# RtrMmmt/MPI-BiCGStab

Hardware: NVIDIA H100
Metric: BiCGStab iterations/sec (higher is better)
Workload: dtype f64

## Files before the change

mpi-bicgstab_b200/csrc/engine.hpp:

```cpp
#pragma once
#include "bicgstab_b200.h"
#include "dev.cuh"
#include "plan.hpp"
#include "spmv.cuh"
#include "vec.cuh"
#include "mega.cuh"

#include <cstdio>
#include <cstdlib>
#include <functional>
#include <initializer_list>
#include <map>
#include <string>
#include <vector>

namespace bicg {

[[noreturn]] void fatal(const char *fmt, ...);
#define BICG_CUDA(call)                                                                              \
    do {                                                                                             \
        cudaError_t e_ = (call);                                                                     \
        if (e_ != cudaSuccess)                                                                       \
            ::bicg::fatal("bicgstab_b200: CUDA error %s at %s:%d: %s", cudaGetErrorName(e_), __FILE__, \
                          __LINE__, cudaGetErrorString(e_));                                          \
// ... 74 lines not shown
    std::vector<Deferred> deferred;
    std::multimap<size_t, void *> pool;
    std::map<void *, size_t> live;
    size_t pool_bytes = 0;
    struct ArenaRec { char *ptr; size_t bytes; unsigned long long id; cudaIpcMemHandle_t handle; };
    std::multimap<size_t, ArenaRec> arena_pool;
    std::map<std::pair<int, unsigned long long>, void *> peer_maps;
    unsigned long long next_arena_id = 1;
    void release_arenas();
    void host_allgather(const void *send, void *recv, size_t bytes);
    void h2d(void *dst, const void *src, size_t bytes);
    struct Stager { cudaStream_t st = nullptr; cudaEvent_t ev[2] = {nullptr, nullptr}; cudaEvent_t done = nullptr; char *buf[2] = {nullptr, nullptr}; };
    std::vector<Stager> stagers;
    int stage_threads = 4;
};
Context &ctx();
void load_config_from_env(Config &c);
int  set_option(Config &c, const char *key, const char *value);


struct SpmvPlan {
    int kind = 0, lanes = 1, threads = 256, stages = 3, cap = 0, grid = 0, ctas_per_sm = 1;
    size_t smem = 0;
    int ntiles = 0;
    int *d_tile_row = nullptr;
    unsigned *d_tile_nz = nullptr;
    double ms = 0.0;
};

struct MegaPlan {
    bool ok = false;
    int threads = 512, lanes = 1, stages = 2, cap = 0, grid = 0;
    size_t smem = 0;
    size_t res_smem = 0;
    int ntiles = 0;
    int *d_tile_row = nullptr;
    unsigned *d_tile_nz = nullptr;
    int *d_cta_tile = nullptr;
    int4 *d_cta_dep = nullptr;
    unsigned short *d_col16 = nullptr;
    bool stream_codes = true;
    int *d_tile_flag = nullptr;
    bool chunked = false;
    std::vector<int> cta_row;
};

}

struct bicg_matrix {
    int rank = 0, world = 1;
    int n_loc = 0, n_glob = 0;
    size_t nnz = 0;
    unsigned max_row = 0;
    double mean_row = 0.0;
    double *d_val = nullptr;
    unsigned *d_col = nullptr;
    unsigned *d_ptr = nullptr;
    bicg::SpmvPlan plan;
    bicg::MegaPlan mega;
    bicg::MegaSync *d_msync = nullptr;
    bicg::MegaSync *peer_msync[bicg::MAX_RANKS] = {};
    unsigned long long *d_ll = nullptr;
    long long ll_stride = 0;
    unsigned long long *peer_ll[bicg::MAX_RANKS] = {};
    long long peer_ll_stride[bicg::MAX_RANKS] = {};
    unsigned long long *d_trace = nullptr;
    int ghost_off = 0;
    int n_ghost = 0;
    long long vstride = 0;
    std::vector<int> recv_runs;
    char *arena = nullptr;
    size_t arena_bytes = 0;
    unsigned long long arena_id = 0;
// ... 73 lines not shown
```

mpi-bicgstab_b200/csrc/matrix.cu:

```cuda
#include "engine.hpp"

#include <algorithm>
#include <climits>
#include <cmath>
#include <cstdarg>
#include <cstring>
#include <ctime>
#include <thread>

namespace bicg {

void fatal(const char *fmt, ...)
{
    va_list ap;
    va_start(ap, fmt);
    vfprintf(stderr, fmt, ap);
    va_end(ap);
    fputc('\n', stderr);
    exit(1);
}

namespace {

enum class Parse { Int, Double, Spmv };
// ... 431 lines not shown
    if (mean_row <= 20.0) return 1;
    if (mean_row <= 40.0) return 4;
    if (mean_row <= 128.0) return 8;
    return 32;
}

static void build_mega_plan(bicg_matrix *m, const unsigned *h_ptr, const std::vector<unsigned char> &row_extra)
{
    Context &c = ctx();
    MegaPlan &mp = m->mega;
    mp.ok = false;
    if (m->n_loc < 1) return;
    const int G = std::min(c.sm_count, MEGA_MAX_CTAS);
    const long long SMEM_MAX = 222 * 1024;
    const int lanes = c.cfg.mega_lanes > 0 ? c.cfg.mega_lanes : mega_lanes_for(m->mean_row);
    if (lanes != 1 && c.cfg.mega != 2 && c.cfg.mega_lanes == 0) return;
    for (int threads : {512, 256}) {
        if (c.cfg.mega_threads && c.cfg.mega_threads != threads) continue;
        if (!mega_has_variant(threads, lanes)) continue;
        const int rpt = threads / lanes;
        std::vector<int> tile_row, cta_tile, tile_flag;
        std::vector<unsigned> tile_nz;
        const int cap_limit = (int)(((SMEM_MAX / 2 - (long long)(rpt + 8) * 4) / 12) / 32 * 32) - 64;
        const unsigned max_tile_nnz = plan_cta_tiles(h_ptr, m->n_loc, G, rpt, row_extra.empty() ? nullptr : row_extra.data(),
                                                     c.cfg.boundary_weight, tile_row, cta_tile, cap_limit, &tile_nz, &tile_flag, c.cfg.row_weight);
        const int cap = round_up((long long)max_tile_nnz + 16, 32);
        const long long stage = (long long)cap * 12 + (long long)(rpt + 8) * 4;
        int stages = (int)std::min<long long>(4, SMEM_MAX / stage);
        if (stages < 2) continue;
        bool chunked = false;
        for (int f : tile_flag) chunked = chunked || f != 0;
        mp.chunked = chunked;
        mp.threads = threads; mp.lanes = lanes; mp.stages = stages; mp.cap = cap; mp.grid = G;
        mp.smem = mega_smem_bytes(cap, stages, threads, lanes);
        mp.res_smem = 0;
        if (lanes == 1 && !chunked) {
            size_t need = 0;
            for (int g = 0; g < G; ++g) {
                const int r0 = tile_row[(size_t)cta_tile[(size_t)g]], r1 = tile_row[(size_t)cta_tile[(size_t)g + 1]];
                need = std::max(need, mega_resident_bytes(h_ptr[r1] - h_ptr[r0], r1 - r0));
            }
            if (need <= (size_t)SMEM_MAX) mp.res_smem = std::max<size_t>(need, 16);
        }
        mp.ntiles = (int)tile_row.size() - 1;
        mp.cta_row.assign((size_t)G + 1, m->n_loc);
        for (int g = 0; g <= G; ++g) mp.cta_row[(size_t)g] = tile_row[(size_t)cta_tile[(size_t)g]];
        mp.d_tile_row = (decltype(mp.d_tile_row))c.dev_alloc(tile_row.size() * sizeof(int));
        mp.d_tile_nz = (decltype(mp.d_tile_nz))c.dev_alloc(tile_nz.size() * sizeof(unsigned));
        mp.d_cta_tile = (decltype(mp.d_cta_tile))c.dev_alloc(cta_tile.size() * sizeof(int));
        mp.d_cta_dep = (decltype(mp.d_cta_dep))c.dev_alloc((size_t)G * sizeof(int4));
        mp.d_tile_flag = nullptr;
        if (chunked) {
            mp.d_tile_flag = (int *)c.dev_alloc(tile_flag.size() * sizeof(int));
            BICG_CUDA(cudaMemcpy(mp.d_tile_flag, tile_flag.data(), tile_flag.size() * sizeof(int), cudaMemcpyHostToDevice));
        }
        BICG_CUDA(cudaMemcpy(mp.d_tile_row, tile_row.data(), tile_row.size() * sizeof(int), cudaMemcpyHostToDevice));
        BICG_CUDA(cudaMemcpy(mp.d_tile_nz, tile_nz.data(), tile_nz.size() * sizeof(unsigned), cudaMemcpyHostToDevice));
        BICG_CUDA(cudaMemcpy(mp.d_cta_tile, cta_tile.data(), cta_tile.size() * sizeof(int), cudaMemcpyHostToDevice));
        launch_mega_dep(m->d_col, m->d_ptr, mp.d_tile_row, mp.d_cta_tile, G, m->ghost_off, mp.d_cta_dep, c.stream);
        BICG_CUDA(cudaGetLastError());
        const size_t pad = 16;
        mp.d_col16 = (unsigned short *)c.dev_alloc((m->nnz + pad) * sizeof(unsigned short));
        BICG_CUDA(cudaMemsetAsync(mp.d_col16 + m->nnz, 0, pad * sizeof(unsigned short), c.stream));
        launch_mega_code(m->d_col, m->d_ptr, mp.d_tile_row, mp.d_cta_tile, G, m->ghost_off, mp.d_cta_dep, mp.d_col16, c.stream);
        BICG_CUDA(cudaGetLastError());
        mp.ok = true;
        if (c.cfg.verbose)
            fprintf(stderr, "[bicg mega r%d] threads=%d lanes=%d stages=%d cap=%d tiles=%d smem=%zu resident_smem=%zu\n", m->rank, threads, lanes,
                    stages, cap, mp.ntiles, mp.smem, mp.res_smem);
        return;
    }
}

__global__ void __launch_bounds__(256) merge_rows_kernel(int n_loc, const unsigned *__restrict__ dptr, const unsigned *__restrict__ optr,
                                                         const double *__restrict__ dval, const unsigned *__restrict__ dcol,
                                                         const double *__restrict__ oval, const unsigned *__restrict__ ocol,
                                                         const int *__restrict__ runs , int nruns, int ghost_off,
                                                         double *__restrict__ mval, unsigned *__restrict__ mcol)
{
    for (int i = blockIdx.x * blockDim.x + threadIdx.x; i < n_loc; i += gridDim.x * blockDim.x) {
        const unsigned d0 = dptr[i], d1 = dptr[i + 1], o0 = optr[i], o1 = optr[i + 1];
        unsigned k = d0 + o0;
        for (unsigned j = d0; j < d1; ++j, ++k) { mval[k] = dval[j]; mcol[k] = dcol[j]; }
        for (unsigned j = o0; j < o1; ++j, ++k) {
            const int gc = (int)ocol[j];
            int a = 0, b = nruns;
            while (b - a > 1) { const int mid = (a + b) >> 1; if (runs[4 * mid] <= gc) a = mid; else b = mid; }
            mval[k] = oval[j];
            mcol[k] = (unsigned)(ghost_off + runs[4 * a + 3] + (gc - runs[4 * a]));
        }
    }
}

void Context::release_arenas()
{
    if (world > 1 && (!arena_pool.empty() || !peer_maps.empty())) {
        int token = 0; std::vector<int> all((size_t)world);
        if (ready) cudaStreamSynchronize(stream);
        host_allgather(&token, all.data(), sizeof(int));
        for (auto &kv : peer_maps) cudaIpcCloseMemHandle(kv.second);
        peer_maps.clear();
        host_allgather(&token, all.data(), sizeof(int));
// ... 239 lines not shown
        int oks[MAX_RANKS] = {};
        BICG_CUDA(cudaMemcpy(oks, m->d_msync->st.plan_ok, sizeof(oks), cudaMemcpyDeviceToHost));
        for (int p = 0; p < m->world; ++p) if (!oks[p]) m->mega.ok = false;
    }
    return m;
}

double matrix_upload_ms(bicg_matrix *m)
{
    if (m->ev_upload0) {
        float ms = 0.f;
        if (cudaEventSynchronize(m->ev_upload1) == cudaSuccess && cudaEventElapsedTime(&ms, m->ev_upload0, m->ev_upload1) == cudaSuccess)
            m->upload_ms = ms;
        cudaEventDestroy(m->ev_upload0); cudaEventDestroy(m->ev_upload1);
        m->ev_upload0 = m->ev_upload1 = nullptr;
    }
    return m->upload_ms;
}

void matrix_destroy(bicg_matrix *m)
{
    if (!m) return;
    Context &c = ctx();
    if (c.ready) cudaStreamSynchronize(c.stream);
    (void)matrix_upload_ms(m);
    for (auto it = c.cache.begin(); it != c.cache.end();) {
        if (it->second == m) it = c.cache.erase(it); else ++it;
    }
    for (int g = 0; g < 4; ++g) if (m->graph[g]) cudaGraphExecDestroy(m->graph[g]);
    for (int s = 0; s < m->npush; ++s) c.dev_free(m->d_push_runs[s]);
    free_plan(m->plan);
    c.dev_free(m->d_trace);
    c.dev_free(m->mega.d_tile_row); c.dev_free(m->mega.d_tile_nz); c.dev_free(m->mega.d_cta_tile); c.dev_free(m->mega.d_cta_dep);
    c.dev_free(m->mega.d_col16); c.dev_free(m->mega.d_tile_flag);
    if (m->hist_extra) cudaFree(m->hist_extra);
    c.dev_free(m->d_val); c.dev_free(m->d_col); c.dev_free(m->d_ptr);
    if (m->world > 1) c.arena_pool.emplace(m->arena_bytes, Context::ArenaRec{m->arena, m->arena_bytes, m->arena_id, m->arena_handle});
    else c.dev_free(m->arena);
    delete m;
}

static uint64_t block_fingerprint(const CSR_Matrix *b, uint64_t h)
{
    auto mix = [&](uint64_t v) { h = (h ^ v) * 0x100000001b3ull; };
    if (!b) { mix(0x9e3779b97f4a7c15ull); return h; }
    mix(b->nz); mix(b->rows); mix(b->cols);
    const size_t S = 8192;
    if (b->nz && b->val && b->col) {
        const size_t step = std::max<size_t>(1, b->nz / S);
        for (size_t i = 0; i < b->nz; i += step) {
            uint64_t bits; memcpy(&bits, &b->val[i], 8);
            mix(bits); mix(b->col[i]);
        }
        uint64_t bits; memcpy(&bits, &b->val[b->nz - 1], 8);
        mix(bits); mix(b->col[b->nz - 1]);
    }
    if (b->ptr) {
        const size_t np1 = (size_t)b->rows + 1, step = std::max<size_t>(1, np1 / S);
        for (size_t i = 0; i < np1; i += step) mix(b->ptr[i]);
        mix(b->ptr[b->rows]);
    }
    return h;
}
static uint64_t host_fingerprint(const CSR_Matrix *diag, const CSR_Matrix *offd, bool with_offd)
{
    uint64_t h = block_fingerprint(diag, 0xcbf29ce484222325ull);
    return with_offd ? block_fingerprint(offd, h) : h;
// ... 28 lines not shown
```

mpi-bicgstab_b200/csrc/mega.cu:

```cuda
#include "mega.cuh"
#include "vec_body.cuh"

namespace bicg {

namespace {

constexpr int RED_THREADS = MEGA_MAX_CTAS;
constexpr int RED_WARPS = RED_THREADS / 32;
struct StageHdr { int row0, row1; unsigned a0; int rowa; unsigned lo, hi; int flag; int pad_; };

__device__ __forceinline__ unsigned long long l2_evict_first_policy()
{
    unsigned long long pol;
    asm volatile("createpolicy.fractional.L2::evict_first.b64 %0, 1.0;" : "=l"(pol));
    return pol;
}
__device__ __forceinline__ void tma_load_1d_hint(unsigned dst_smem, const void *src, unsigned bytes, unsigned bar,
                                                 unsigned long long pol)
{
    asm volatile("cp.async.bulk.shared::cluster.global.mbarrier::complete_tx::bytes.L2::cache_hint [%0], [%1], %2, [%3], %4;"
                 ::"r"(dst_smem), "l"(src), "r"(bytes), "r"(bar), "l"(pol) : "memory");
}
__device__ __forceinline__ void poll_pause(unsigned spins)
{
// ... 5 lines not shown
{
    const int lane = threadIdx.x & 31, warp = threadIdx.x >> 5;
    constexpr int NW = CT / 32;
#pragma unroll
    for (int k = 0; k < N; ++k) v[k] = warp_sum(v[k]);
    nbar(1, CT);
    if (lane == 0) {
#pragma unroll
        for (int k = 0; k < N; ++k) scratch[warp * N + k] = v[k];
    }
    nbar(1, CT);
    if (warp == 0) {
#pragma unroll
        for (int k = 0; k < N; ++k) {
            double t = (lane < NW) ? scratch[lane * N + k] : 0.0;
            v[k] = warp_sum(t);
        }
    }
}

enum Epi : int { EPI_NONE = 0, EPI_RH_Y, EPI_QY_YY, EPI_CA4 };

struct MegaShared {
    Scalars sc;
    double tot[MAIL_VALS];
    double red[RED_WARPS][MAIL_VALS];
    double contrib[MAX_RANKS][MAIL_VALS];
    double scratch[32 * MAX_DOTS];
    unsigned long long full_bar[4], empty_bar[4];
    StageHdr hdr[4];
    volatile int flags[4];
};

struct ColWindow { bool ok; unsigned ospan; int obase, gbase; };
__device__ __forceinline__ ColWindow col_window(int4 dep, int ghost_off)
{
    ColWindow w;
    const bool own = dep.x <= dep.y, gh = dep.z <= dep.w;
    w.ospan = own ? (unsigned)(dep.y - dep.x + 1) : 0u;
    const unsigned gspan = gh ? (unsigned)(dep.w - dep.z + 1) : 0u;
    w.ok = w.ospan + gspan <= 65536u;
    w.obase = own ? dep.x : 0;
    w.gbase = ghost_off + (gh ? dep.z : 0) - (int)w.ospan;
    return w;
}
__device__ __forceinline__ unsigned short col_encode(const ColWindow &w, int ghost_off, unsigned c)
{
    return (unsigned short)((int)c < ghost_off ? (int)c - w.obase : (int)c - w.gbase);
}
__device__ __forceinline__ unsigned col_decode(const ColWindow &w, unsigned code)
{
    return code + (unsigned)(code < w.ospan ? w.obase : w.gbase);
}

struct ResidentPlan { bool on; int row_lo, rows; unsigned nz_lo, nnz; ColWindow w; };
__device__ __forceinline__ ResidentPlan resident_plan(const MegaArgs &a, int t0, int t1, int lanes)
{
    ResidentPlan p;
    p.on = false; p.row_lo = 0; p.rows = 0; p.nz_lo = 0u; p.nnz = 0u;
    p.w = col_window(a.cta_dep[blockIdx.x], a.ghost_off);
    if (!a.resident || lanes != 1 || t1 <= t0 || a.tile_flag != nullptr) return p;
    p.row_lo = a.tile_row[t0];
    p.rows = a.tile_row[t1] - p.row_lo;
    if (p.rows <= 0) return p;
    p.nz_lo = a.ptr[p.row_lo];
    p.nnz = a.ptr[p.row_lo + p.rows] - p.nz_lo;
    if (mega_resident_bytes(p.nnz, p.rows) > (size_t)a.smem_bytes) return p;
    p.on = p.w.ok;
    return p;
}
__device__ __forceinline__ bool streams_codes(const MegaArgs &a, const ResidentPlan &rp, int my_tiles)
{
    return a.stream_codes && a.col16 != nullptr && my_tiles > 0 && !rp.on && rp.w.ok;
}

template <int CT, int LANES>
struct Mega {
    static constexpr int RPT = CT / LANES, PROW = RPT + PROW_PAD, NCW = CT / 32, UNR = (LANES == 1) ? 16 : 8;
    static_assert(CT >= RED_THREADS, "the slot reduction uses one thread per CTA slot");

    const MegaArgs &a;
    MegaShared &sh;
    unsigned char *dyn;
    int tid, lane, my_tiles, row_lo, row_hi;
    unsigned vis;
    unsigned gen;
    unsigned red_epoch;
    unsigned posted_gen;
    unsigned long long halo_epoch;
    int dep_lo, dep_hi;
    unsigned push_slots;
    int ghost_lo, ghost_hi;
    int gs_lo, gs_hi;
    bool reads_ghost;
    bool is_reducer;
    size_t stage_bytes;
    int trace_it, trace_who;
    bool resident;
    bool coded;
    ResidentPlan rp;
    const double *rs_val; const unsigned short *rs_col; const unsigned *rs_ptr;

    __device__ Mega(const MegaArgs &args, MegaShared &s) : a(args), sh(s) {}

    __device__ bool stop_now() const { return sh.sc.done != 0 || sh.sc.error != 0; }
    __device__ void fail() { sh.flags[3] = 1; }
// ... 258 lines not shown
            while (j < e) {
                double xv[U];
#pragma unroll
                for (int u = 0; u < U; ++u) {
                    const unsigned c = rs_col[min(min(j + (unsigned)u, e - 1u), last)];
                    xv[u] = ld_coherent((c < ospan ? xo : xg) + c);
                }
#pragma unroll
                for (int u = 0; u < U; ++u) {
                    const double v = rs_val[min(min(j + (unsigned)u, e - 1u), last)];
                    if (j + (unsigned)u < e) acc = fma(v, xv[u], acc);
                }
                j += (unsigned)U;
            }
            row_done<EPI>(row, acc, e0, e1, e2, e3, y, dot);
        }
    }

    template <int EPI, bool CODED>
    __device__ void spmv_impl(const double *x, double *y, double (&dot)[4])
    {
        const int stages = a.stages, cap = a.cap;
        const int sub = tid % LANES, row_in_tile = tid / LANES;
        const ColWindow w = rp.w;
        double carry = 0.0;
        for (int lt = 0; lt < my_tiles; ++lt, ++vis) {
            const int s = (int)(vis % (unsigned)stages);
            mbar_wait(smem_u32(&sh.full_bar[s]), (vis / (unsigned)stages) & 1u);
            const unsigned char *st = dyn + (size_t)s * stage_bytes;
            const double   *sval = reinterpret_cast<const double *>(st);
            const unsigned *scol = reinterpret_cast<const unsigned *>(sval + cap);
            const unsigned short *scode = reinterpret_cast<const unsigned short *>(scol);
            const unsigned *sptr = scol + cap;
            auto column = [&](unsigned idx) { return CODED ? col_decode(w, scode[idx]) : scol[idx]; };
            const StageHdr h = sh.hdr[s];
            if (h.flag != 0) {
                double part[1] = {0.0};
                for (unsigned jj = h.lo + (unsigned)tid; jj < h.hi; jj += 4u * CT) {
                    double pv[4], px[4];
#pragma unroll
                    for (int u = 0; u < 4; ++u) {
                        const unsigned idx = min(jj + (unsigned)(u * CT), h.hi - 1u);
                        pv[u] = sval[idx]; px[u] = ld_coherent(x + column(idx));
                    }
#pragma unroll
                    for (int u = 0; u < 4; ++u)
                        if (jj + (unsigned)(u * CT) < h.hi) part[0] = fma(pv[u], px[u], part[0]);
                }
                cblock_sum<1, CT>(part, sh.scratch);
                if (tid == 0) sh.red[0][0] = part[0];
                nbar(1, CT);
                carry += sh.red[0][0];
                if (h.flag == 2) {
                    if (tid == 0) {
                        double e0 = 0.0, e1 = 0.0, e2 = 0.0, e3 = 0.0;
                        epi_load<EPI>(h.row0, e0, e1, e2, e3);
                        row_done<EPI>(h.row0, carry, e0, e1, e2, e3, y, dot);
                    }
                    carry = 0.0;
                }
                __syncwarp();
                if (lane == 0) mbar_arrive(smem_u32(&sh.empty_bar[s]));
                continue;
            }
            const int row = h.row0 + row_in_tile;
            const bool valid = row < h.row1;
            int j = 0, e = 0;
            double e0 = 0.0, e1 = 0.0, e2 = 0.0, e3 = 0.0;
            if (valid) {
                j = (int)(sptr[row - h.rowa] - h.a0) + sub;
                e = (int)(sptr[row - h.rowa + 1] - h.a0);
                if (sub == 0) epi_load<EPI>(row, e0, e1, e2, e3);
            }
            const double acc = row_product<LANES, UNR>(sval, column, x, j, e);
            if (valid && sub == 0) row_done<EPI>(row, acc, e0, e1, e2, e3, y, dot);
            __syncwarp();
            if (lane == 0) mbar_arrive(smem_u32(&sh.empty_bar[s]));
        }
    }

    template <int PH>
    __device__ void vec(double *dot)
    {
        Coef c;
        c.al = sh.sc.alpha; c.be = sh.sc.beta; c.om = sh.sc.omega;
        c.nbo = -c.be * c.om;
        const int hi2 = row_lo + ((row_hi - row_lo) & ~1);
        int i = row_lo + 2 * tid;
        for (; i + 2 * CT < hi2; i += 4 * CT) body<PH, Pairs<2, 2 * CT>>(a.v, i, c, dot);
        for (; i < hi2; i += 2 * CT) body<PH, Pairs<1, 2 * CT>>(a.v, i, c, dot);
        if (tid == 0 && hi2 < row_hi) body<PH, Contig<1>>(a.v, hi2, c, dot);
    }
    __device__ void sync_local(bool all)
    {
        double d0[1] = {0.0};
        arrive<0>(d0, true);
        if (!all) { wait_nbr(); return; }
        wait_all();
        if (tid < RED_THREADS) {
            nbar(2, RED_THREADS);
            if (tid < 32) fence_gpu();
        }
        nbar(1, CT);
        if (sh.flags[3]) { if (tid == 0) { sh.sc.error = 1; sh.sc.done = 1; } nbar(1, CT); }
// ... 216 lines not shown
                spmv<EPI_NONE>(a.v.r, a.v.w, d4);
                nbar(1, CT);
                vec<PH_RR_DOTS>(d5);
            }
            post<5>(d5, V_W, LL_W);
            spmv<EPI_NONE>(a.v.w, a.v.t, d4);
            complete<5>(FIN_CAPIPE_END, true);
            if (stop_now()) break;
        }
    }
};

template <int CT, int LANES>
__global__ void __launch_bounds__(CT + 32, 1) bicg_mega_kernel(const __grid_constant__ MegaArgs a)
{
    using M = Mega<CT, LANES>;
    extern __shared__ __align__(128) unsigned char dyn_smem[];
    __shared__ __align__(16) MegaShared sh;

    const int tid = threadIdx.x;
    const int stages = a.stages, cap = a.cap;
    if (tid == 0) {
        for (int s = 0; s < stages; ++s) {
            mbar_init(smem_u32(&sh.full_bar[s]), 1u);
            mbar_init(smem_u32(&sh.empty_bar[s]), (unsigned)M::NCW);
        }
        sh.flags[0] = sh.flags[1] = sh.flags[2] = sh.flags[3] = 0;
        mbar_fence_init();
    }
    __syncthreads();

    const int t0 = a.cta_tile[blockIdx.x], t1 = a.cta_tile[blockIdx.x + 1];
    const int my_tiles = t1 - t0;
    const size_t stage_bytes = (size_t)cap * 12 + (size_t)M::PROW * 4;

    if (tid >= CT) {
        const ResidentPlan rp = tid == CT ? resident_plan(a, t0, t1, LANES) : ResidentPlan{};
        if (tid == CT && my_tiles > 0 && !rp.on) {
            volatile int *flags = sh.flags;
            const unsigned long long pol = l2_evict_first_policy();
            const bool coded = streams_codes(a, rp, my_tiles);
            const unsigned al = coded ? 7u : 3u, cbytes = coded ? 2u : 4u;
            const void *cols = coded ? (const void *)a.col16 : (const void *)a.col;
            unsigned v = 0;
            bool stop = false;
            for (;; ++v) {
                const int s = (int)(v % (unsigned)stages);
                if (v >= (unsigned)stages) {
                    const unsigned par = (v / (unsigned)stages - 1u) & 1u;
                    while (!mbar_try_wait(smem_u32(&sh.empty_bar[s]), par)) {
                        if (flags[1]) { stop = true; break; }
                    }
                }
                if (stop || flags[1]) break;
                const int t = t0 + (int)(v % (unsigned)my_tiles);
                const int row0 = a.tile_row[t], row1 = a.tile_row[t + 1];
                const unsigned p0 = a.tile_nz[t], p1 = a.tile_nz[t + 1];
                const auto [a0, cnt, rowa, cntp] = tile_window(row0, row1, p0, p1, al);
                unsigned char *st = dyn_smem + (size_t)s * stage_bytes;
                double   *sval = reinterpret_cast<double *>(st);
                unsigned *scol = reinterpret_cast<unsigned *>(sval + cap);
                unsigned *sptr = scol + cap;
                sh.hdr[s] = StageHdr{row0, row1, a0, rowa, p0 - a0, p1 - a0, a.tile_flag ? a.tile_flag[t] : 0, 0};
                const unsigned bar = smem_u32(&sh.full_bar[s]);
                mbar_arrive_expect_tx(bar, cnt * (8u + cbytes) + (unsigned)cntp * 4u);
                if (cnt) {
                    const void *csrc = (const char *)cols + (size_t)a0 * cbytes;
                    tma_load_1d_hint(smem_u32(sval), a.val + a0, cnt * 8u, bar, pol);
                    tma_load_1d_hint(smem_u32(scol), csrc, cnt * cbytes, bar, pol);
                }
                tma_load_1d(smem_u32(sptr), a.ptr + rowa, (unsigned)cntp * 4u, bar);
            }
            const unsigned consumed = (unsigned)flags[2];
            for (unsigned w = consumed; w < v; ++w)
                mbar_wait(smem_u32(&sh.full_bar[w % (unsigned)stages]), (w / (unsigned)stages) & 1u);
        }
    } else {
        M m(a, sh);
        m.dyn = dyn_smem; m.tid = tid; m.lane = tid & 31; m.my_tiles = my_tiles; m.vis = 0u; m.stage_bytes = stage_bytes;
        m.row_lo = a.tile_row[t0]; m.row_hi = a.tile_row[t1];
        m.trace_it = 0;
        m.trace_who = blockIdx.x == 0 ? 0 : (blockIdx.x == gridDim.x / 2 ? 1 : -1);
        m.gen = a.sync->st.gen; m.red_epoch = a.sync->st.red_epoch; m.halo_epoch = a.sync->st.halo_epoch;
        m.posted_gen = m.gen;
        if (tid == 0) sh.sc = *a.sc;

        const int4 dep = a.cta_dep[blockIdx.x];
        const int G = (int)gridDim.x;
        auto cta_of_row = [&](int r) {
            int lo = 0, hi = G;
            while (lo < hi) { const int mid = (lo + hi) >> 1; if (a.tile_row[a.cta_tile[mid]] <= r) lo = mid + 1; else hi = mid; }
            return lo - 1;
        };
        m.dep_lo = 1; m.dep_hi = 0;
        if (dep.x <= dep.y) { m.dep_lo = max(0, cta_of_row(dep.x)); m.dep_hi = min(G - 1, cta_of_row(dep.y)); }
        m.reads_ghost = a.comm.world > 1 && dep.z <= dep.w;
        m.ghost_lo = m.reads_ghost ? dep.z : 0; m.ghost_hi = m.reads_ghost ? dep.w + 1 : 0;
        m.is_reducer = (int)blockIdx.x == G / 2;
        m.gs_lo = m.gs_hi = 0;
        if (a.comm.world > 1) {
            const int ng = a.n_ghost;
            const int chunk = ((ng + G - 1) / G + 15) & ~15;
            m.gs_lo = min(ng, (int)blockIdx.x * chunk);
            m.gs_hi = min(ng, m.gs_lo + chunk);
        }
        m.push_slots = 0u;
        if (a.comm.world > 1) {
            PushDesc pd;
            pd.npeers = 1;
            for (int s = 0; s < a.push.npeers; ++s) {
                pd.runs[0] = a.push.runs[s]; pd.nruns[0] = a.push.nruns[s];
                if (m.row_hi > m.row_lo && push_touches(pd, m.row_lo, m.row_hi)) m.push_slots |= 1u << s;
            }
        }
        m.rp = resident_plan(a, t0, t1, LANES);
        m.resident = m.rp.on;
        m.coded = streams_codes(a, m.rp, my_tiles);
        if (m.resident) {
            const size_t nnzp = ((size_t)m.rp.nnz + 7u) & ~(size_t)7u;
            double *sv = reinterpret_cast<double *>(dyn_smem);
            unsigned short *sc16 = reinterpret_cast<unsigned short *>(sv + nnzp);
            unsigned *sp = reinterpret_cast<unsigned *>(sc16 + nnzp);
            for (unsigned i = (unsigned)tid; i < m.rp.nnz; i += (unsigned)CT) {
                sv[i] = a.val[m.rp.nz_lo + i];
                sc16[i] = a.col16[m.rp.nz_lo + i];
            }
            for (int r = tid; r <= m.rp.rows; r += CT) sp[r] = a.ptr[m.rp.row_lo + r] - m.rp.nz_lo;
            m.rs_val = sv; m.rs_col = sc16; m.rs_ptr = sp;
            if (tid == 0) atomicAdd(&a.sync->st.resident_ctas, 1);
        }
        if (m.coded && tid == 0) atomicAdd(&a.sync->st.coded_ctas, 1);
        nbar(1, CT);
        if (a.comm.world > 1 && (m.reads_ghost || m.gs_hi > m.gs_lo)) {
            if (tid < 32 && !halo_wait_epoch(a.comm, sh.sc.halo_epoch) && tid == 0) { sh.sc.error = 1; sh.sc.done = 1; }
            if (tid < 32) fence_sys();
            nbar(1, CT);
        }
        if (!m.stop_now()) {
            if (a.method == 0) { if (a.comm.world > 1) m.run_bicgstab_multi(); else m.run_bicgstab(); }
            else if (a.method == 1) m.run_ca();
            else m.run_pipe(a.method == 3);
        }
        nbar(1, CT);
        if (tid == 0) {
            sh.flags[2] = (int)m.vis; __threadfence_block(); sh.flags[1] = 1;
            if (blockIdx.x == 0) {
                *a.sc = sh.sc;
                a.sync->st.gen = m.gen; a.sync->st.red_epoch = m.red_epoch; a.sync->st.halo_epoch = m.halo_epoch;
            } else if (sh.sc.error) a.sc->error = 1;
        }
// ... 22 lines not shown
    if (threadIdx.x == 0) dep[blockIdx.x] = make_int4(s[0], s[1], s[2], s[3]);
}

__global__ void __launch_bounds__(256) mega_code_kernel(const unsigned *__restrict__ col, const unsigned *__restrict__ ptr,
                                                        const int *__restrict__ tile_row, const int *__restrict__ cta_tile,
                                                        int ghost_off, const int4 *__restrict__ dep, unsigned short *__restrict__ col16)
{
    const ColWindow w = col_window(dep[blockIdx.x], ghost_off);
    if (!w.ok) return;
    const int r0 = tile_row[cta_tile[blockIdx.x]], r1 = tile_row[cta_tile[blockIdx.x + 1]];
    if (r1 <= r0) return;
    const unsigned e0 = ptr[r0], e1 = ptr[r1];
    for (unsigned j = e0 + threadIdx.x; j < e1; j += blockDim.x) col16[j] = col_encode(w, ghost_off, col[j]);
}

template <int CT, int LANES>
cudaError_t launch(const MegaArgs &a, int grid, size_t smem, cudaStream_t st)
{
    void *params[1] = {(void *)&a};
    return cudaLaunchCooperativeKernel((const void *)bicg_mega_kernel<CT, LANES>, dim3(grid), dim3(CT + 32), params, smem, st);
}
template <int CT, int LANES>
cudaError_t set_attr()
{
    cudaFuncAttributes fa;
    cudaError_t e = cudaFuncGetAttributes(&fa, bicg_mega_kernel<CT, LANES>);
    if (e != cudaSuccess) return e;
    return cudaFuncSetAttribute(bicg_mega_kernel<CT, LANES>, cudaFuncAttributeMaxDynamicSharedMemorySize,
                                227 * 1024 - (int)fa.sharedSizeBytes);
}

}

size_t mega_smem_bytes(int cap, int stages, int threads, int lanes)
{
    return (size_t)stages * ((size_t)cap * 12u + (size_t)(threads / lanes + PROW_PAD) * 4u);
}

bool mega_has_variant(int threads, int lanes)
{
    if (threads == 256) return lanes == 1;
    return threads == 512 && (lanes == 1 || lanes == 4 || lanes == 8 || lanes == 32);
}

int mega_setup_attributes()
{
    cudaError_t e;
    if ((e = set_attr<256, 1>()) != cudaSuccess) return (int)e;
    if ((e = set_attr<512, 1>()) != cudaSuccess) return (int)e;
    if ((e = set_attr<512, 4>()) != cudaSuccess) return (int)e;
    if ((e = set_attr<512, 8>()) != cudaSuccess) return (int)e;
    if ((e = set_attr<512, 32>()) != cudaSuccess) return (int)e;
    return 0;
}

int launch_mega(int threads, int lanes, int grid, size_t smem, const MegaArgs &a, cudaStream_t st)
{
    if (threads == 256 && lanes == 1) return (int)launch<256, 1>(a, grid, smem, st);
    if (threads != 512) return (int)cudaErrorInvalidValue;
    switch (lanes) {
    case 1:  return (int)launch<512, 1>(a, grid, smem, st);
    case 4:  return (int)launch<512, 4>(a, grid, smem, st);
    case 8:  return (int)launch<512, 8>(a, grid, smem, st);
    case 32: return (int)launch<512, 32>(a, grid, smem, st);
    default: return (int)cudaErrorInvalidValue;
    }
}

void launch_mega_dep(const unsigned *col, const unsigned *ptr, const int *tile_row, const int *cta_tile, int grid,
// ... 13 lines not shown
```

mpi-bicgstab_b200/csrc/mega.cuh:

```cuda
#pragma once
#include "dev.cuh"
#include "vec.cuh"

namespace bicg {

constexpr int MEGA_MAX_CTAS   = 160;
constexpr int MEGA_RING       = 8;
constexpr int MEGA_SLOT_WORDS = 16;

struct alignas(128) MegaSlot { unsigned long long w[MEGA_SLOT_WORDS]; };

struct alignas(128) MegaState {
    unsigned gen;
    unsigned red_epoch;
    unsigned long long halo_epoch;
    int plan_ok[MAX_RANKS];
    int resident_ctas;
    int coded_ctas;
};

struct MegaSync {
    MegaState st;
    MegaSlot  slot[MEGA_RING][MEGA_MAX_CTAS];
    MegaSlot  mail[2][MAX_RANKS];
};

struct PushPlan {
    int npeers;
    int peer[MAX_RANKS - 1];
    const PushRun *runs[MAX_RANKS - 1];
    int nruns[MAX_RANKS - 1];
    unsigned long long *ll_dst[MAX_RANKS - 1];
    long long ll_stride[MAX_RANKS - 1];
};

enum LLRegion : int { LL_S0 = 0, LL_S1, LL_R, LL_P, LL_Z, LL_X, LL_W, LL_REGIONS };

constexpr int MEGA_TRACE_ITERS = 256, MEGA_TRACE_SLOTS = 16;

struct MegaArgs {
    Scalars *sc;
    double  *hist;
    CommDev  comm;
    MegaSync *sync;
    MegaSlot *peer_mail[MAX_RANKS];
    int n_ghost;
    const int4 *cta_dep;
    const double   *val;
    const unsigned *col;
    const unsigned short *col16;
    const unsigned *ptr;
    const int      *tile_row;
    const unsigned *tile_nz;
    const int      *cta_tile;
    const int      *tile_flag;
    int cap, stages;
    int ghost_off;
    int resident;
    int stream_codes;
    int smem_bytes;
    double *vec_base; long long vstride;
    VecPtrs v;
    PushPlan push;
    const unsigned long long *ll;
    long long ll_stride;
    int method;
    int krr, nrr;
    unsigned long long *snap;
    int snap_iter;
    unsigned long long *trace;
};

int    launch_mega(int threads, int lanes, int grid, size_t smem, const MegaArgs &a, cudaStream_t st);
int    mega_setup_attributes();
bool   mega_has_variant(int threads, int lanes);
size_t mega_smem_bytes(int cap, int stages, int threads, int lanes);
__host__ __device__ inline size_t mega_resident_bytes(unsigned nnz, int rows)
{
    const size_t nnzp = ((size_t)nnz + 7u) & ~(size_t)7u;
    return nnzp * 10u + ((size_t)rows + 1u) * 4u;
}
void   launch_mega_dep(const unsigned *col, const unsigned *ptr, const int *tile_row, const int *cta_tile, int grid,
                       int ghost_off, int4 *dep, cudaStream_t st);
void   launch_mega_code(const unsigned *col, const unsigned *ptr, const int *tile_row, const int *cta_tile, int grid,
                        int ghost_off, const int4 *dep, unsigned short *col16, cudaStream_t st);

}
```

mpi-bicgstab_b200/csrc/solve.cu:

```cuda
#include "engine.hpp"
#include "vec_body.cuh"

#include <algorithm>
#include <cmath>
#include <cstring>

namespace bicg {

namespace {

__global__ void reset_state_kernel(Scalars *s, double tol, int max_iter)
{
    s->rTr = s->rTr_old = s->rTs = s->rTy = s->yTy = s->rTw = s->wTw = s->rTz = 0.0;
    s->dot_r = s->dot_zero = 0.0;
    s->alpha = s->beta = s->omega = 0.0;
    s->tol2 = tol * tol;
    for (int k = 0; k < MAX_DOTS; ++k) s->pend[k] = 0.0;
    s->k = 0; s->max_iter = max_iter; s->done = 0; s->converged = 0; s->error = 0; s->ticket = 0u;
}

__global__ void fill_kernel(double *p, int n, double v)
{
    for (int i = blockIdx.x * blockDim.x + threadIdx.x; i < n; i += gridDim.x * blockDim.x) p[i] = v;
}
// ... 84 lines not shown
        if (b >= depth) {
            const int o = (b - depth) % Context::FLAG_RING;
            BICG_CUDA(cudaEventSynchronize(ring[(size_t)o]));
            if (c.h_flags[o]) break;
        }
        enqueue_batch(b);
        const int o = b % Context::FLAG_RING;
        BICG_CUDA(cudaMemcpyAsync(&c.h_flags[o], d_done, sizeof(int), cudaMemcpyDeviceToHost, c.stream));
        if (!ring[(size_t)o]) BICG_CUDA(cudaEventCreateWithFlags(&ring[(size_t)o], cudaEventDisableTiming));
        BICG_CUDA(cudaEventRecord(ring[(size_t)o], c.stream));
    }
    for (cudaEvent_t e : ring) if (e) cudaEventDestroy(e);
}

void print_times(double seconds, double iters)
{
    printf("Total time   : %e [sec.] \n", seconds);
    printf("Avg time/iter: %e [sec.] \n", seconds / iters);
    fflush(stdout);
}

namespace {

struct Seq : PhaseLauncher {
    using PhaseLauncher::PhaseLauncher;

    bool mega(int method, int krr, int nrr)
    {
        MegaArgs a{};
        a.sc = m->d_sc; a.hist = m->d_hist; a.comm = m->comm; a.sync = m->d_msync;
        for (int p = 0; p < MAX_RANKS; ++p) a.peer_mail[p] = &m->peer_msync[p]->mail[0][0];
        a.n_ghost = m->n_ghost; a.cta_dep = m->mega.d_cta_dep;
        a.val = m->d_val; a.col = m->d_col; a.col16 = m->mega.d_col16; a.ptr = m->d_ptr;
        a.stream_codes = m->mega.stream_codes ? 1 : 0;
        a.tile_row = m->mega.d_tile_row; a.tile_nz = m->mega.d_tile_nz; a.cta_tile = m->mega.d_cta_tile;
        a.tile_flag = m->mega.d_tile_flag;
        a.cap = m->mega.cap; a.stages = m->mega.stages;
        a.ghost_off = m->ghost_off;
        size_t smem = m->mega.smem;
        a.resident = (c.cfg.resident && m->mega.res_smem) ? 1 : 0;
        if (a.resident) smem = std::max(smem, m->mega.res_smem);
        a.smem_bytes = (int)smem;
        a.vec_base = m->vec_base; a.vstride = m->vstride;
        a.v = ptrs();
        a.push.npeers = m->world > 1 ? m->npush : 0;
        for (int s = 0; s < a.push.npeers; ++s) {
            const int d = m->push_peer[s];
            a.push.peer[s] = d;
            a.push.runs[s] = m->d_push_runs[s];
            a.push.nruns[s] = m->push_nruns[s];
            a.push.ll_dst[s] = m->peer_ll[d];
            a.push.ll_stride[s] = m->peer_ll_stride[d];
        }
        a.ll = m->d_ll; a.ll_stride = m->ll_stride;
        a.method = method; a.krr = krr; a.nrr = nrr;
        a.trace = m->d_trace;
        a.snap = m->d_trace ? m->d_trace + (size_t)2 * MEGA_TRACE_ITERS * MEGA_TRACE_SLOTS : nullptr;
        a.snap_iter = 50;
        BICG_CUDA(cudaMemsetAsync(&m->d_msync->st.resident_ctas, 0, sizeof(int), c.stream));
        BICG_CUDA(cudaMemsetAsync(&m->d_msync->st.coded_ctas, 0, sizeof(int), c.stream));
        int rc = launch_mega(m->mega.threads, m->mega.lanes, m->mega.grid, smem, a, c.stream);
        if (rc) {
            (void)cudaGetLastError();
            if (m->world > 1) fatal("bicgstab_b200: rank %d could not launch the persistent kernel: %s", m->rank,
                                    cudaGetErrorString((cudaError_t)rc));
            if (c.cfg.verbose) fprintf(stderr, "[bicg] persistent kernel not launched (%s); using the per-phase kernels\n",
                                       cudaGetErrorString((cudaError_t)rc));
            m->mega.ok = false;
            return false;
        }
        ++launches; ++c.launches;
        return true;
// ... 440 lines not shown
```

Baseline: 3603.

## Stream 16-bit row offsets and pack coded stages tighter in mega SpMV

When the persistent kernel streams 16-bit column codes, it now also streams precomputed 16-bit per-row offsets relative to each tile's aligned start, in place of 32-bit CSR row pointers. Stage layout shrinks so column codes use 2 bytes each, and dynamic shared memory is sized by a coded variant when every CTA's column window fits. This reduces TMA bytes per tile and shared memory footprint, which may allow more overlap, at the cost of host-side setup, an extra device array, and a branch for the last row's end offset.

Result: faster. 3664 (median of 6 runs) (+1.7%).

```diff
diff --git a/mpi-bicgstab_b200/csrc/engine.hpp b/mpi-bicgstab_b200/csrc/engine.hpp
--- a/mpi-bicgstab_b200/csrc/engine.hpp
+++ b/mpi-bicgstab_b200/csrc/engine.hpp
@@ -130,6 +130,7 @@
     bool ok = false;
     int threads = 512, lanes = 1, stages = 2, cap = 0, grid = 0;
     size_t smem = 0;
+    size_t smem_coded = 0;
     size_t res_smem = 0;
     int ntiles = 0;
     int *d_tile_row = nullptr;
@@ -137,6 +138,7 @@
     int *d_cta_tile = nullptr;
     int4 *d_cta_dep = nullptr;
     unsigned short *d_col16 = nullptr;
+    unsigned short *d_off16 = nullptr;
     bool stream_codes = true;
     int *d_tile_flag = nullptr;
     bool chunked = false;
diff --git a/mpi-bicgstab_b200/csrc/matrix.cu b/mpi-bicgstab_b200/csrc/matrix.cu
--- a/mpi-bicgstab_b200/csrc/matrix.cu
+++ b/mpi-bicgstab_b200/csrc/matrix.cu
@@ -487,7 +487,7 @@
         for (int f : tile_flag) chunked = chunked || f != 0;
         mp.chunked = chunked;
         mp.threads = threads; mp.lanes = lanes; mp.stages = stages; mp.cap = cap; mp.grid = G;
-        mp.smem = mega_smem_bytes(cap, stages, threads, lanes);
+        mp.smem = mega_smem_bytes(cap, stages, threads, lanes, false);
         mp.res_smem = 0;
         if (lanes == 1 && !chunked) {
             size_t need = 0;
@@ -514,15 +514,40 @@
         BICG_CUDA(cudaMemcpy(mp.d_cta_tile, cta_tile.data(), cta_tile.size() * sizeof(int), cudaMemcpyHostToDevice));
         launch_mega_dep(m->d_col, m->d_ptr, mp.d_tile_row, mp.d_cta_tile, G, m->ghost_off, mp.d_cta_dep, c.stream);
         BICG_CUDA(cudaGetLastError());
+        std::vector<int4> dep((size_t)G);
+        BICG_CUDA(cudaMemcpyAsync(dep.data(), mp.d_cta_dep, (size_t)G * sizeof(int4), cudaMemcpyDeviceToHost, c.stream));
+        BICG_CUDA(cudaStreamSynchronize(c.stream));
+        bool all_coded = true;
+        for (int g = 0; g < G; ++g)
+            if (cta_tile[(size_t)g + 1] > cta_tile[(size_t)g]) all_coded = all_coded && col_window(dep[(size_t)g], m->ghost_off).ok;
+        mp.smem_coded = all_coded ? mega_smem_bytes(cap, stages, threads, lanes, true) : 0;
         const size_t pad = 16;
         mp.d_col16 = (unsigned short *)c.dev_alloc((m->nnz + pad) * sizeof(unsigned short));
         BICG_CUDA(cudaMemsetAsync(mp.d_col16 + m->nnz, 0, pad * sizeof(unsigned short), c.stream));
         launch_mega_code(m->d_col, m->d_ptr, mp.d_tile_row, mp.d_cta_tile, G, m->ghost_off, mp.d_cta_dep, mp.d_col16, c.stream);
         BICG_CUDA(cudaGetLastError());
+        {
+            std::vector<unsigned short> off((size_t)m->n_loc + 16, 0);
+            bool fits = true;
+            for (size_t t = 0; t + 1 < tile_row.size(); ++t) {
+                if (!tile_flag.empty() && tile_flag[t] != 0) continue;
+                const unsigned a0 = tile_nz[t] & ~7u;
+                for (int r = tile_row[t]; r < tile_row[t + 1]; ++r) {
+                    fits = fits && h_ptr[r] - a0 <= 0xffffu;
+                    off[(size_t)r] = (unsigned short)(h_ptr[r] - a0);
+                }
+            }
+            mp.d_off16 = nullptr;
+            if (fits) {
+                mp.d_off16 = (unsigned short *)c.dev_alloc(off.size() * sizeof(unsigned short));
+                BICG_CUDA(cudaMemcpy(mp.d_off16, off.data(), off.size() * sizeof(unsigned short), cudaMemcpyHostToDevice));
+            }
+            if (!mp.d_off16) mp.smem_coded = 0;
+        }
         mp.ok = true;
         if (c.cfg.verbose)
-            fprintf(stderr, "[bicg mega r%d] threads=%d lanes=%d stages=%d cap=%d tiles=%d smem=%zu resident_smem=%zu\n", m->rank, threads, lanes,
-                    stages, cap, mp.ntiles, mp.smem, mp.res_smem);
+            fprintf(stderr, "[bicg mega r%d] threads=%d lanes=%d stages=%d cap=%d tiles=%d smem=%zu coded_smem=%zu resident_smem=%zu\n",
+                    m->rank, threads, lanes, stages, cap, mp.ntiles, mp.smem, mp.smem_coded, mp.res_smem);
         return;
     }
 }
@@ -828,7 +853,7 @@
     free_plan(m->plan);
     c.dev_free(m->d_trace);
     c.dev_free(m->mega.d_tile_row); c.dev_free(m->mega.d_tile_nz); c.dev_free(m->mega.d_cta_tile); c.dev_free(m->mega.d_cta_dep);
-    c.dev_free(m->mega.d_col16); c.dev_free(m->mega.d_tile_flag);
+    c.dev_free(m->mega.d_col16); c.dev_free(m->mega.d_tile_flag); c.dev_free(m->mega.d_off16);
     if (m->hist_extra) cudaFree(m->hist_extra);
     c.dev_free(m->d_val); c.dev_free(m->d_col); c.dev_free(m->d_ptr);
     if (m->world > 1) c.arena_pool.emplace(m->arena_bytes, Context::ArenaRec{m->arena, m->arena_bytes, m->arena_id, m->arena_handle});
diff --git a/mpi-bicgstab_b200/csrc/mega.cu b/mpi-bicgstab_b200/csrc/mega.cu
--- a/mpi-bicgstab_b200/csrc/mega.cu
+++ b/mpi-bicgstab_b200/csrc/mega.cu
@@ -61,18 +61,6 @@
     volatile int flags[4];
 };
 
-struct ColWindow { bool ok; unsigned ospan; int obase, gbase; };
-__device__ __forceinline__ ColWindow col_window(int4 dep, int ghost_off)
-{
-    ColWindow w;
-    const bool own = dep.x <= dep.y, gh = dep.z <= dep.w;
-    w.ospan = own ? (unsigned)(dep.y - dep.x + 1) : 0u;
-    const unsigned gspan = gh ? (unsigned)(dep.w - dep.z + 1) : 0u;
-    w.ok = w.ospan + gspan <= 65536u;
-    w.obase = own ? dep.x : 0;
-    w.gbase = ghost_off + (gh ? dep.z : 0) - (int)w.ospan;
-    return w;
-}
 __device__ __forceinline__ unsigned short col_encode(const ColWindow &w, int ghost_off, unsigned c)
 {
     return (unsigned short)((int)c < ghost_off ? (int)c - w.obase : (int)c - w.gbase);
@@ -101,6 +89,10 @@
 __device__ __forceinline__ bool streams_codes(const MegaArgs &a, const ResidentPlan &rp, int my_tiles)
 {
     return a.stream_codes && a.col16 != nullptr && my_tiles > 0 && !rp.on && rp.w.ok;
+}
+__device__ __forceinline__ size_t stage_bytes_of(const MegaArgs &a, bool coded, int prow)
+{
+    return mega_stage_bytes(a.cap, prow, coded);
 }
 
 template <int CT, int LANES>
@@ -425,6 +417,7 @@
             const unsigned *scol = reinterpret_cast<const unsigned *>(sval + cap);
             const unsigned short *scode = reinterpret_cast<const unsigned short *>(scol);
             const unsigned *sptr = scol + cap;
+            const unsigned short *soff = scode + cap;
             auto column = [&](unsigned idx) { return CODED ? col_decode(w, scode[idx]) : scol[idx]; };
             const StageHdr h = sh.hdr[s];
             if (h.flag != 0) {
@@ -461,8 +454,13 @@
             int j = 0, e = 0;
             double e0 = 0.0, e1 = 0.0, e2 = 0.0, e3 = 0.0;
             if (valid) {
-                j = (int)(sptr[row - h.rowa] - h.a0) + sub;
-                e = (int)(sptr[row - h.rowa + 1] - h.a0);
+                if (CODED) {
+                    j = (int)soff[row - h.rowa] + sub;
+                    e = row + 1 < h.row1 ? (int)soff[row - h.rowa + 1] : (int)h.hi;
+                } else {
+                    j = (int)(sptr[row - h.rowa] - h.a0) + sub;
+                    e = (int)(sptr[row - h.rowa + 1] - h.a0);
+                }
                 if (sub == 0) epi_load<EPI>(row, e0, e1, e2, e3);
             }
             const double acc = row_product<LANES, UNR>(sval, column, x, j, e);
@@ -745,7 +743,6 @@
 
     const int t0 = a.cta_tile[blockIdx.x], t1 = a.cta_tile[blockIdx.x + 1];
     const int my_tiles = t1 - t0;
-    const size_t stage_bytes = (size_t)cap * 12 + (size_t)M::PROW * 4;
 
     if (tid >= CT) {
         const ResidentPlan rp = tid == CT ? resident_plan(a, t0, t1, LANES) : ResidentPlan{};
@@ -753,6 +750,7 @@
             volatile int *flags = sh.flags;
             const unsigned long long pol = l2_evict_first_policy();
             const bool coded = streams_codes(a, rp, my_tiles);
+            const size_t stage_bytes = stage_bytes_of(a, coded, M::PROW);
             const unsigned al = coded ? 7u : 3u, cbytes = coded ? 2u : 4u;
             const void *cols = coded ? (const void *)a.col16 : (const void *)a.col;
             unsigned v = 0;
@@ -769,20 +767,23 @@
                 const int t = t0 + (int)(v % (unsigned)my_tiles);
                 const int row0 = a.tile_row[t], row1 = a.tile_row[t + 1];
                 const unsigned p0 = a.tile_nz[t], p1 = a.tile_nz[t + 1];
-                const auto [a0, cnt, rowa, cntp] = tile_window(row0, row1, p0, p1, al);
+                auto [a0, cnt, rowa, cntp] = tile_window(row0, row1, p0, p1, al);
+                if (coded) { rowa = row0 & ~7; cntp = ((row1 + 7) & ~7) - rowa; }
                 unsigned char *st = dyn_smem + (size_t)s * stage_bytes;
                 double   *sval = reinterpret_cast<double *>(st);
-                unsigned *scol = reinterpret_cast<unsigned *>(sval + cap);
-                unsigned *sptr = scol + cap;
+                unsigned char *scol = reinterpret_cast<unsigned char *>(sval + cap);
+                unsigned char *sptr = scol + (size_t)cap * cbytes;
+                const unsigned pbytes = coded ? 2u : 4u;
                 sh.hdr[s] = StageHdr{row0, row1, a0, rowa, p0 - a0, p1 - a0, a.tile_flag ? a.tile_flag[t] : 0, 0};
                 const unsigned bar = smem_u32(&sh.full_bar[s]);
-                mbar_arrive_expect_tx(bar, cnt * (8u + cbytes) + (unsigned)cntp * 4u);
+                mbar_arrive_expect_tx(bar, cnt * (8u + cbytes) + (unsigned)cntp * pbytes);
                 if (cnt) {
                     const void *csrc = (const char *)cols + (size_t)a0 * cbytes;
                     tma_load_1d_hint(smem_u32(sval), a.val + a0, cnt * 8u, bar, pol);
                     tma_load_1d_hint(smem_u32(scol), csrc, cnt * cbytes, bar, pol);
                 }
-                tma_load_1d(smem_u32(sptr), a.ptr + rowa, (unsigned)cntp * 4u, bar);
+                const void *psrc = coded ? (const void *)(a.off16 + rowa) : (const void *)(a.ptr + rowa);
+                tma_load_1d(smem_u32(sptr), psrc, (unsigned)cntp * pbytes, bar);
             }
             const unsigned consumed = (unsigned)flags[2];
             for (unsigned w = consumed; w < v; ++w)
@@ -790,7 +791,7 @@
         }
     } else {
         M m(a, sh);
-        m.dyn = dyn_smem; m.tid = tid; m.lane = tid & 31; m.my_tiles = my_tiles; m.vis = 0u; m.stage_bytes = stage_bytes;
+        m.dyn = dyn_smem; m.tid = tid; m.lane = tid & 31; m.my_tiles = my_tiles; m.vis = 0u;
         m.row_lo = a.tile_row[t0]; m.row_hi = a.tile_row[t1];
         m.trace_it = 0;
         m.trace_who = blockIdx.x == 0 ? 0 : (blockIdx.x == gridDim.x / 2 ? 1 : -1);
@@ -829,6 +830,7 @@
         m.rp = resident_plan(a, t0, t1, LANES);
         m.resident = m.rp.on;
         m.coded = streams_codes(a, m.rp, my_tiles);
+        m.stage_bytes = stage_bytes_of(a, m.coded, M::PROW);
         if (m.resident) {
             const size_t nnzp = ((size_t)m.rp.nnz + 7u) & ~(size_t)7u;
             double *sv = reinterpret_cast<double *>(dyn_smem);
@@ -917,9 +919,9 @@
 
 }
 
-size_t mega_smem_bytes(int cap, int stages, int threads, int lanes)
-{
-    return (size_t)stages * ((size_t)cap * 12u + (size_t)(threads / lanes + PROW_PAD) * 4u);
+size_t mega_smem_bytes(int cap, int stages, int threads, int lanes, bool coded)
+{
+    return (size_t)stages * mega_stage_bytes(cap, threads / lanes + PROW_PAD, coded);
 }
 
 bool mega_has_variant(int threads, int lanes)
diff --git a/mpi-bicgstab_b200/csrc/mega.cuh b/mpi-bicgstab_b200/csrc/mega.cuh
--- a/mpi-bicgstab_b200/csrc/mega.cuh
+++ b/mpi-bicgstab_b200/csrc/mega.cuh
@@ -50,6 +50,7 @@
     const unsigned *col;
     const unsigned short *col16;
     const unsigned *ptr;
+    const unsigned short *off16;
     const int      *tile_row;
     const unsigned *tile_nz;
     const int      *cta_tile;
@@ -74,7 +75,24 @@
 int    launch_mega(int threads, int lanes, int grid, size_t smem, const MegaArgs &a, cudaStream_t st);
 int    mega_setup_attributes();
 bool   mega_has_variant(int threads, int lanes);
-size_t mega_smem_bytes(int cap, int stages, int threads, int lanes);
+__host__ __device__ inline size_t mega_stage_bytes(int cap, int prow, bool coded)
+{
+    return (size_t)cap * (coded ? 10u : 12u) + (size_t)prow * 4u;
+}
+size_t mega_smem_bytes(int cap, int stages, int threads, int lanes, bool coded);
+
+struct ColWindow { bool ok; unsigned ospan; int obase, gbase; };
+__host__ __device__ inline ColWindow col_window(int4 dep, int ghost_off)
+{
+    ColWindow w;
+    const bool own = dep.x <= dep.y, gh = dep.z <= dep.w;
+    w.ospan = own ? (unsigned)(dep.y - dep.x + 1) : 0u;
+    const unsigned gspan = gh ? (unsigned)(dep.w - dep.z + 1) : 0u;
+    w.ok = w.ospan + gspan <= 65536u;
+    w.obase = own ? dep.x : 0;
+    w.gbase = ghost_off + (gh ? dep.z : 0) - (int)w.ospan;
+    return w;
+}
 __host__ __device__ inline size_t mega_resident_bytes(unsigned nnz, int rows)
 {
     const size_t nnzp = ((size_t)nnz + 7u) & ~(size_t)7u;
diff --git a/mpi-bicgstab_b200/csrc/solve.cu b/mpi-bicgstab_b200/csrc/solve.cu
--- a/mpi-bicgstab_b200/csrc/solve.cu
+++ b/mpi-bicgstab_b200/csrc/solve.cu
@@ -140,12 +140,13 @@
         for (int p = 0; p < MAX_RANKS; ++p) a.peer_mail[p] = &m->peer_msync[p]->mail[0][0];
         a.n_ghost = m->n_ghost; a.cta_dep = m->mega.d_cta_dep;
         a.val = m->d_val; a.col = m->d_col; a.col16 = m->mega.d_col16; a.ptr = m->d_ptr;
-        a.stream_codes = m->mega.stream_codes ? 1 : 0;
+        a.off16 = m->mega.d_off16;
+        a.stream_codes = (m->mega.stream_codes && m->mega.d_off16) ? 1 : 0;
         a.tile_row = m->mega.d_tile_row; a.tile_nz = m->mega.d_tile_nz; a.cta_tile = m->mega.d_cta_tile;
         a.tile_flag = m->mega.d_tile_flag;
         a.cap = m->mega.cap; a.stages = m->mega.stages;
         a.ghost_off = m->ghost_off;
-        size_t smem = m->mega.smem;
+        size_t smem = (a.stream_codes && m->mega.smem_coded) ? m->mega.smem_coded : m->mega.smem;
         a.resident = (c.cfg.resident && m->mega.res_smem) ? 1 : 0;
         if (a.resident) smem = std::max(smem, m->mega.res_smem);
         a.smem_bytes = (int)smem;
```
